# LiyaoTang/contrastBoundary

Hardware: AMD Instinct MI355X
Metric: points/sec through KNN+group+KPConv+CBL block, S3DIS N=40960 K=16 (higher is better)
Workload: dtype f32

## Files before the change

### contrastboundary_amd/csrc/knn_grid.hip

```cpp
#include "cbl_common.h"
#include <cstdlib>
#include "grid_core.h"
#include <knn_wave.h>

int cbl_knn_exact_worklist(int b, int m, int K, const float* xyz, const float* new_xyz, const int* offset,
                           const int* new_offset, int* idx, float* dist2,
                           const int* worklist, const int* worklist_count, int max_work, hipStream_t st,
                           const void* grids, const int* cell_start, const void* sorted);

namespace {

constexpr int GRID_MAX_K = 64;
constexpr int CELLS_PER_POINT = 2;
constexpr int CELLS_PER_CLOUD = 64;

struct Workspace {
    CblGrid* grids;
    int* counters;
    unsigned* bbox;
    int* cell_count;
    int* cell_start;
    int* cell_local;
    int* tile_sum;
    int* pt_cell;
// ... 245 lines not shown
    sort_cx<LEX>(d, i, l8, lane, PermRowMir());    sort_cx<LEX>(d, i, l4, lane, PermSwzXor4());  sort_cx<LEX>(d, i, l2, lane, PermQuadXor2());
    sort_cx<LEX>(d, i, l1, lane, PermQuadXor1());
    sort_cx<LEX>(d, i, l16, lane, PermSwzMir32()); sort_cx<LEX>(d, i, l8, lane, PermRowRor8());  sort_cx<LEX>(d, i, l4, lane, PermSwzXor4());
    sort_cx<LEX>(d, i, l2, lane, PermQuadXor2());  sort_cx<LEX>(d, i, l1, lane, PermQuadXor1());
    sort_cx<LEX>(d, i, l32, lane, PermMir64());    sort_cx<LEX>(d, i, l16, lane, PermSwzXor16()); sort_cx<LEX>(d, i, l8, lane, PermRowRor8());
    sort_cx<LEX>(d, i, l4, lane, PermSwzXor4());   sort_cx<LEX>(d, i, l2, lane, PermQuadXor2()); sort_cx<LEX>(d, i, l1, lane, PermQuadXor1());
}
__device__ __forceinline__ float rl_f(float v, int l) { return __int_as_float(__builtin_amdgcn_readlane(__float_as_int(v), l)); }
template <int G> __device__ __forceinline__ float group_min_nonneg(float f)
{
    int v = __float_as_int(f);
    v = min(v, dppx_i<0xB1>(v)); v = min(v, dppx_i<0x4E>(v)); v = min(v, dppx_i<0x141>(v)); v = min(v, dppx_i<0x140>(v));
    if constexpr (G == 32) v = min(v, __builtin_amdgcn_ds_swizzle(v, 0x401f));
    if constexpr (G == 64) v = min(min(__builtin_amdgcn_readlane(v, 0), __builtin_amdgcn_readlane(v, 16)),
                                   min(__builtin_amdgcn_readlane(v, 32), __builtin_amdgcn_readlane(v, 48)));
    return __int_as_float(v);
}

template <int G, bool SELF, bool LEX>
__global__ __launch_bounds__(256) void knn_grid_group_kernel(int b, int m, int K, const float* __restrict__ new_xyz,
                                                             const int* __restrict__ offset, const int* __restrict__ new_offset,
                                                             const CblGrid* __restrict__ grids, const int* __restrict__ cell_start,
                                                             const float4* __restrict__ sorted, int* __restrict__ idx, float* __restrict__ dist2,
                                                             int* __restrict__ worklist, int* __restrict__ counters, int set_exact)
{
    constexpr int QPW = 64 / G;
    using mask_t = unsigned long long;
    const int lane = threadIdx.x & 63;
    const int gl = lane & (G - 1);
    const int grp = lane / G;
    const int wave_global = (blockIdx.x * 256 + threadIdx.x) >> 6;
    const int t = wave_global * QPW + grp;
    const bool live = t < m;
    const int tt = live ? t : m - 1;

    int q; float qx, qy, qz;
    if (SELF) { const float4 s = sorted[tt]; q = __float_as_int(s.w); qx = s.x; qy = s.y; qz = s.z; }
    else      { q = tt; qx = new_xyz[3 * q]; qy = new_xyz[3 * q + 1]; qz = new_xyz[3 * q + 2]; }
    const int c = cbl_cloud_of(q, SELF ? offset : new_offset, b);
    const CblGrid g = grids[c];
    const float uqx = cbl_u(qx, g.ox, g.inv_cs), uqy = cbl_u(qy, g.oy, g.inv_cs), uqz = cbl_u(qz, g.oz, g.inv_cs);
    const int cx = cbl_cell_coord(uqx, g.nx), cy = cbl_cell_coord(uqy, g.ny), cz = cbl_cell_coord(uqz, g.nz);

    float ed = INFINITY; int ei = -1;
    float rejmin = INFINITY;
    int evict = 0x7f800000;
    const int last_src = ((lane & ~(G - 1)) + K - 1) << 2;
    bool done = !live;

    int rs9 = 0, re9 = 0;
    if (!done && gl < 9) {
        const int o = (int)((0xa82091645ull >> (4 * gl)) & 0xFull);
        const int y = cy + (o & 3) - 1, z = cz + (o >> 2) - 1;
        if (y >= 0 && y < g.ny && z >= 0 && z < g.nz) {
            const int row = g.cell_base + g.nx * (y + g.ny * z);
            rs9 = cell_start[row + max(cx - 1, 0)]; re9 = cell_start[row + min(cx + 1, g.nx - 1) + 1];
        }
    }
    const int grp_src = (lane & ~(G - 1)) << 2;

    for (int r = 1;; r++) {
        const int side = 2 * r + 1;
        for (int ri = 0; ri < side * side; ri++) {
            int dy, dz;
            if (r == 1) { const int o = (int)((0xa82091645ull >> (4 * ri)) & 0xFull); dy = (o & 3) - 1; dz = (o >> 2) - 1; }
            else        { dz = ri / side - r; dy = ri % side - r; }
            {
                const bool full = (r == 1) || dz == -r || dz == r || dy == -r || dy == r;
                const int nseg = full ? 1 : 2;
                for (int sg = 0; sg < nseg; sg++) {
                    int x0, x1;
                    if (full) { x0 = max(cx - r, 0); x1 = min(cx + r, g.nx - 1); }
                    else      { x0 = x1 = sg ? cx + r : cx - r; }
                    const int y = cy + dy, z = cz + dz;
                    int s = 0, e = 0;
                    if (r == 1) {
                        s = __builtin_amdgcn_ds_bpermute(grp_src + (ri << 2), rs9); e = __builtin_amdgcn_ds_bpermute(grp_src + (ri << 2), re9);
                    } else if (!done && y >= 0 && y < g.ny && z >= 0 && z < g.nz && x0 >= 0 && x1 <= g.nx - 1) {
                        const int row = g.cell_base + g.nx * (y + g.ny * z);
                        s = cell_start[row + x0]; e = cell_start[row + x1 + 1];
                    }
                    for (int p = s; __any(p < e); p += G) {
                        const int pi = p + gl;
                        float d2 = INFINITY; int ci = -1;
                        if (pi < e) {
                            const float4 v = sorted[pi];
                            d2 = cbl_dist2(qx, qy, qz, v.x, v.y, v.z);
                            ci = __float_as_int(v.w);
                        }
                        const float worst = __int_as_float(__builtin_amdgcn_ds_bpermute(last_src, __float_as_int(ed)));
                        const unsigned worst_i = LEX ? (unsigned)__builtin_amdgcn_ds_bpermute(last_src, ei) : 0u;
                        const bool pass = d2 < worst || (LEX && d2 == worst && (unsigned)ci < worst_i);
                        rejmin = __int_as_float(min(__float_as_int(rejmin), pass ? 0x7f800000 : __float_as_int(d2)));
                        if constexpr (!LEX && G <= 32) {
                            unsigned gm = (unsigned)(__ballot(pass) >> (grp * G)) & (G == 32 ? ~0u : ((1u << G) - 1u));
                            const int d2i = __float_as_int(d2);
                            auto step = [&]() {
                                const bool has = gm != 0;
                                const int l = kw_ffbl(gm);
                                gm &= gm - 1;
                                const int src = (l << 2) + grp * (G * 4);
                                int dci = __builtin_amdgcn_ds_bpermute(src, d2i); const int ic = __builtin_amdgcn_ds_bpermute(src, ci);
                                dci = has ? dci : 0x7f800000;
                                const int edi = __float_as_int(ed);
                                int pdi = dpp_shr1_zero<G>(edi), pidx = dpp_shr1_zero<G>(ei);
                                if (G == 32) pdi = gl ? pdi : 0;
                                evict = min(evict, max(edi, dci));
                                ei = (edi > dci) ? ((pdi > dci) ? pidx : ic) : ei;
                                ed = __int_as_float(min(edi, max(pdi, dci)));
                            };
                            while (__any(gm != 0)) {
                                step();
                                if (!__any(gm != 0)) break;
                                step();
                            }
                        } else {
                        mask_t gm = (__ballot(pass) >> (grp * G)) & (G == 64 ? ~0ull : ((1ull << G) - 1ull));
                        while (__any(gm != 0)) {
                            const bool has = gm != 0;
                            const int l = has ? __builtin_ctzll(gm) : 0;
                            gm &= gm - 1;
                            float dc = __shfl(d2, l, G); int ic = __shfl(ci, l, G);
                            if (!has) { dc = INFINITY; ic = -1; }
                            const float pd = dpp_shr1_f<G>(ed); const int pidx = dpp_shr1_i<G>(ei);
                            const bool gt = ed > dc || (LEX && ed == dc && (unsigned)ei > (unsigned)ic);
                            const bool left_gt = (gl > 0) && (pd > dc || (LEX && pd == dc && (unsigned)pidx > (unsigned)ic));
                            if (gl == K - 1) rejmin = fminf(rejmin, gt ? ed : dc);
                            if (gt) { if (left_gt) { ed = pd; ei = pidx; } else { ed = dc; ei = ic; } }
                        }
                        }
                    }
                }
            }
        }
        const float bound2 = cbl_outside_bound2(g, uqx, uqy, uqz, cx, cy, cz, r);
        const float worst = __int_as_float(__builtin_amdgcn_ds_bpermute(last_src, __float_as_int(ed)));
        if (!done) done = (bound2 == INFINITY) || (worst < bound2);
        if (__all(done)) break;
    }

    const float worst = __int_as_float(__builtin_amdgcn_ds_bpermute(last_src, __float_as_int(ed)));
    const float rm = group_min_nonneg<G>(fminf(rejmin, gl == K - 1 ? __int_as_float(evict) : INFINITY));
    const float pd = dpp_shr1_f<G>(ed);
    const bool dup = (gl > 0) && (gl < K) && (ed == pd);
    const mask_t dm = (__ballot(dup) >> (grp * G)) & (G == 64 ? ~0ull : ((1ull << G) - 1ull));
    const bool ok = (worst < INFINITY) && (set_exact == 2 || ((rm != worst) && (set_exact ? !(dm & 2ull) : dm == 0)));
    if (live) {
        if (gl < K) { idx[(size_t)q * K + gl] = ei; dist2[(size_t)q * K + gl] = ed; }
        if (!ok && gl == 0) worklist[atomicAdd(counters, 1)] = q;
    }
}


template <bool SELF, bool LEX>
__global__ __launch_bounds__(256) void knn_grid_wave_kernel(int b, int m, int K, const float* __restrict__ new_xyz,
                                                            const int* __restrict__ offset, const int* __restrict__ new_offset,
                                                            const CblGrid* __restrict__ grids, const int* __restrict__ cell_start,
                                                            const float4* __restrict__ sorted, int* __restrict__ idx, float* __restrict__ dist2,
                                                            int* __restrict__ worklist, int* __restrict__ counters, int set_exact,
                                                            int ks, int* __restrict__ idx_n, float* __restrict__ dist2_n,
                                                            int* __restrict__ worklist_n, int set_exact_n, CblCanon canon)
{
    __shared__ float2 slots[4][64];
    if ((int)blockIdx.x < canon.blocks) {
        grid_order_canon_body(canon.n, canon.pt_cell, cell_start, sorted, canon.order, blockIdx.x, canon.blocks);
        return;
    }
    const int lane = threadIdx.x & 63, wv = threadIdx.x >> 6;
    const int t = __builtin_amdgcn_readfirstlane(((int)blockIdx.x - canon.blocks) * 4 + wv);
    if (t >= m) return;
    int q; float qx, qy, qz;
    if (SELF) { const float4 s = sorted[t]; q = __float_as_int(s.w); qx = s.x; qy = s.y; qz = s.z; }
    else      { q = t; qx = new_xyz[3 * q]; qy = new_xyz[3 * q + 1]; qz = new_xyz[3 * q + 2]; }
    q = __builtin_amdgcn_readfirstlane(q);
    const int c = cbl_cloud_of(q, SELF ? offset : new_offset, b);
    const CblGrid g = grids[c];
    const float uqx = cbl_u(qx, g.ox, g.inv_cs), uqy = cbl_u(qy, g.oy, g.inv_cs), uqz = cbl_u(qz, g.oz, g.inv_cs);
    const int cx = cbl_cell_coord(uqx, g.nx), cy = cbl_cell_coord(uqy, g.ny), cz = cbl_cell_coord(uqz, g.nz);

    int rs = 0, rlen = 0;
    if (lane < 9) {
        const int y = cy + lane % 3 - 1, z = cz + lane / 3 - 1;
        if (y >= 0 && y < g.ny && z >= 0 && z < g.nz) {
            const int row = g.cell_base + g.nx * (y + g.ny * z);
            rs = cell_start[row + max(cx - 1, 0)];
            rlen = cell_start[row + min(cx + 1, g.nx - 1) + 1] - rs;
        }
    }
    int pre[9], delta[9], T = 0;
#pragma unroll
    for (int r = 0; r < 9; r++) {
        const int s_r = __builtin_amdgcn_readlane(rs, r), l_r = __builtin_amdgcn_readlane(rlen, r);
        pre[r] = T; delta[r] = s_r - T; T += l_r;
    }

    float ed = INFINITY; int ei = -1;
    float rejmin = INFINITY;
    bool fast = (T >= K) && (T <= 64 * WV_NB);
    if (fast) {
        float d[WV_NB]; int id[WV_NB];
        int delta_v[9];
#pragma unroll
        for (int r = 0; r < 9; r++) delta_v[r] = kw_in_vgpr(delta[r]);
#pragma unroll
        for (int j0 = 0; j0 < WV_NB; j0 += 4) {
            float4 p[4];
#pragma unroll
            for (int u = 0; u < 4; u++) {
                if ((j0 + u) * 64 < T) {
                    const int v = min((j0 + u) * 64 + lane, T - 1);
                    int dl = delta_v[0];
#pragma unroll
                    for (int r = 1; r < 9; r++) dl = (v >= pre[r]) ? delta_v[r] : dl;
                    p[u] = sorted[v + dl];
                }
            }
#pragma unroll
            for (int u = 0; u < 4; u++) {
                const int j = j0 + u;
                d[j] = INFINITY; id[j] = -1;
                if (j * 64 < T) {
                    const bool in = j * 64 + lane < T;
                    const float dd = cbl_dist2(qx, qy, qz, p[u].x, p[u].y, p[u].z);
                    d[j] = in ? dd : INFINITY; id[j] = in ? __float_as_int(p[u].w) : -1;
                }
            }
        }
        float tau = 3.0e38f;
        if (T > 64) {
            int mxi = 0;
#pragma unroll
            for (int j = 0; j < WV_NB; j++) {
                if ((j + 1) * 64 <= T) mxi = max(mxi, __float_as_int(d[j]));
                else if (j * 64 < T)   mxi = max(mxi, d[j] < INFINITY ? __float_as_int(d[j]) : 0);
            }
            mxi = max(mxi, dppx_i<0xB1>(mxi)); mxi = max(mxi, dppx_i<0x4E>(mxi));
            mxi = max(mxi, dppx_i<0x141>(mxi)); mxi = max(mxi, dppx_i<0x140>(mxi));
            float lo = -1.f, hi = __int_as_float(max(max(__builtin_amdgcn_readlane(mxi, 0), __builtin_amdgcn_readlane(mxi, 16)),
                                                     max(__builtin_amdgcn_readlane(mxi, 32), __builtin_amdgcn_readlane(mxi, 48))));
            const float first = (float)(K + 64) * 0.6f * __builtin_amdgcn_rcpf((float)T);
            fast = false;
            for (int it = 0; it < 40; it++) {
                const float mid = it == 0 ? hi * first : lo + (hi - lo) * 0.5f;
                if (!(mid > lo && mid < hi)) break;
                int cnt = 0;
#pragma unroll
                for (int j = 0; j < WV_NB; j++) if (j * 64 < T) cnt += __popcll(__ballot(d[j] <= mid));
                if (cnt < K) lo = mid; else if (cnt > 64) hi = mid; else { tau = mid; fast = true; break; }
            }
        }
        if (fast) {
            int base = 0;
#pragma unroll
            for (int j = 0; j < WV_NB; j++) {
                if (j * 64 < T) {
                    const bool pass = d[j] <= tau;
                    const unsigned long long mk = __ballot(pass);
                    if (pass) {
                        const int slot = base + __builtin_amdgcn_mbcnt_hi((unsigned)(mk >> 32), __builtin_amdgcn_mbcnt_lo((unsigned)mk, 0));
                        slots[wv][slot] = make_float2(d[j], __int_as_float(id[j]));
                    } else rejmin = fminf(rejmin, d[j]);
                    base += __popcll(mk);
                }
            }
            __builtin_amdgcn_fence(__ATOMIC_RELEASE, "wavefront");
            __builtin_amdgcn_wave_barrier();
            __builtin_amdgcn_fence(__ATOMIC_ACQUIRE, "wavefront");
            float sd = INFINITY; int si = -1;
            if (lane < base) { const float2 v = slots[wv][lane]; sd = v.x; si = __float_as_int(v.y); }
            wave_sort64<LEX>(sd, si, lane);
            if (lane < K) { ed = sd; ei = si; } else rejmin = fminf(rejmin, sd);
        }
    }

    bool done = false;
    int r = 1;
    if (fast) {
        const float bound2 = cbl_outside_bound2(g, uqx, uqy, uqz, cx, cy, cz, 1);
        done = (bound2 == INFINITY) || (rl_f(ed, K - 1) < bound2);
        r = 2;
    }
    for (; !done; r++) {
        const int side = 2 * r + 1;
        for (int ri = 0; ri < side * side; ri++) {
            const int dz = ri / side - r, dy = ri % side - r;
            const bool full = (r == 1) || dz == -r || dz == r || dy == -r || dy == r;
            const int nseg = full ? 1 : 2;
            for (int sg = 0; sg < nseg; sg++) {
                int x0, x1;
                if (full) { x0 = max(cx - r, 0); x1 = min(cx + r, g.nx - 1); }
                else      { x0 = x1 = sg ? cx + r : cx - r; }
                const int y = cy + dy, z = cz + dz;
                int s = 0, e = 0;
                if (y >= 0 && y < g.ny && z >= 0 && z < g.nz && x0 >= 0 && x1 <= g.nx - 1) {
                    const int row = g.cell_base + g.nx * (y + g.ny * z);
                    s = cell_start[row + x0]; e = cell_start[row + x1 + 1];
                }
                s = __builtin_amdgcn_readfirstlane(s); e = __builtin_amdgcn_readfirstlane(e);
                for (int p = s; p < e; p += 64) {
                    const int pi = p + lane;
                    float d2 = INFINITY; int ci = -1;
                    if (pi < e) {
                        const float4 v = sorted[pi];
                        d2 = cbl_dist2(qx, qy, qz, v.x, v.y, v.z);
                        ci = __float_as_int(v.w);
                    }
                    const float worst = rl_f(ed, K - 1); const unsigned worst_i = LEX ? (unsigned)__builtin_amdgcn_readlane(ei, K - 1) : 0u;
                    const bool pass = d2 < worst || (LEX && d2 == worst && (unsigned)ci < worst_i);
                    rejmin = fminf(rejmin, pass ? INFINITY : d2);
                    unsigned long long gm = __ballot(pass);
                    while (gm) {
                        const int l = __builtin_ctzll(gm);
                        gm &= gm - 1;
                        const float dc = rl_f(d2, l); const int ic = __builtin_amdgcn_readlane(ci, l);
                        const float pd = dpp_shr1_f<64>(ed); const int pidx = dpp_shr1_i<64>(ei);
                        const bool gt = ed > dc || (LEX && ed == dc && (unsigned)ei > (unsigned)ic);
                        const bool left_gt = (lane > 0) && (pd > dc || (LEX && pd == dc && (unsigned)pidx > (unsigned)ic));
                        if (lane == K - 1) rejmin = fminf(rejmin, gt ? ed : dc);
                        if (gt) { if (left_gt) { ed = pd; ei = pidx; } else { ed = dc; ei = ic; } }
                    }
                }
            }
        }
        const float bound2 = cbl_outside_bound2(g, uqx, uqy, uqz, cx, cy, cz, r);
        done = (bound2 == INFINITY) || (rl_f(ed, K - 1) < bound2);
    }

    const float worst = rl_f(ed, K - 1);
    const float rm = group_min_nonneg<64>(rejmin);
    const float pd = dpp_shr1_f<64>(ed);
    const bool dup = (lane > 0) && (lane < K) && (ed == pd);
    const bool ok = (worst < INFINITY) && (set_exact == 2 || ((rm != worst) && (set_exact ? !(__ballot(dup) & 2ull) : __ballot(dup) == 0)));
    if (lane < K) { idx[(size_t)q * K + lane] = ei; dist2[(size_t)q * K + lane] = ed; }
    if (!ok && lane == 0) worklist[atomicAdd(counters, 1)] = q;
    if (idx_n) {
        if (lane < ks) { idx_n[(size_t)q * ks + lane] = ei; dist2_n[(size_t)q * ks + lane] = ed; }
        const bool bad = (lane > 0 && lane <= ks && ed == pd && (lane == ks || lane == 1 || !set_exact_n)) || (lane == ks - 1 && !(ed < 1e10f));
        if (__ballot(bad) != 0ull && lane == 0) worklist_n[atomicAdd(counters + 1, 1)] = q;
    }
}

template <int G>
void launch_query(bool self, int b, int m, int K, const float* new_xyz, const int* offset, const int* new_offset, const Workspace& w,
                  int* idx, float* dist2, int set_exact, hipStream_t st)
{
    const long long waves = ((long long)m + (64 / G) - 1) / (64 / G);
    const dim3 grid(cbl_div_up(waves, 4)), block(256);
#define CBL_LAUNCH_GROUP(SELF_, LEX_) hipLaunchKernelGGL((knn_grid_group_kernel<G, SELF_, LEX_>), grid, block, 0, st, b, m, K, new_xyz, offset, new_offset, w.grids, \
                                                         w.cell_start, w.sorted, idx, dist2, w.worklist, w.counters, set_exact)
    if (set_exact == 2) { if (self) CBL_LAUNCH_GROUP(true, true); else CBL_LAUNCH_GROUP(false, true); }
    else                { if (self) CBL_LAUNCH_GROUP(true, false); else CBL_LAUNCH_GROUP(false, false); }
#undef CBL_LAUNCH_GROUP
}


template <int G>
__device__ __forceinline__ unsigned long long group_min_u64(unsigned long long v)
{
#pragma unroll
    for (int s = G / 2; s >= 1; s >>= 1) {
        const unsigned lo = __shfl_xor((unsigned)v, s, G), hi = __shfl_xor((unsigned)(v >> 32), s, G);
        const unsigned long long o = ((unsigned long long)hi << 32) | lo;
        v = o < v ? o : v;
    }
    return v;
}

__device__ __forceinline__ unsigned long long radius_key_lds(int t, int total, int c1, int c2, int c3, int c4, int c5, int c6, int c7, int c8, const int* __restrict__ otab,
                                                              float qx, float qy, float qz, float r2, const float4* __restrict__ sorted)
{
    const bool have = t < total;
    const int r = (t >= c1) + (t >= c2) + (t >= c3) + (t >= c4) + (t >= c5) + (t >= c6) + (t >= c7) + (t >= c8);
    const int o = otab[r];
    const float4 v = sorted[have ? t + o : 0];
    const float d2 = cbl_dist2(qx, qy, qz, v.x, v.y, v.z);
    return (have && d2 < r2) ? (((unsigned long long)__float_as_uint(d2) << 32) | (unsigned)__float_as_int(v.w)) : ~0ull;
}

template <int G, int U>
__global__ __launch_bounds__(256) void radius_group_kernel(int b, int nq, int ns_total, int limit, float r2, const float* __restrict__ queries,
                                                           const int* __restrict__ q_offset, const CblGrid* __restrict__ grids,
                                                           const int* __restrict__ cell_start, const float4* __restrict__ sorted,
                                                           int* __restrict__ out, int* __restrict__ counts, int* __restrict__ max_count)
{
    constexpr int QPW = 64 / G, CAP = 2 * G, NBF = G >= 64 ? 2 : 4;
    using mask_t = unsigned long long;
    using key_t = unsigned long long;
    constexpr key_t NONE = ~0ull;
    __shared__ key_t slots[4 * QPW][CAP];
    __shared__ int otabs[4 * QPW][U][12];
    const int lane = threadIdx.x & 63, gl = lane & (G - 1), grp = lane / G;
    key_t* S = slots[(threadIdx.x >> 6) * QPW + grp];
    const int wave_global = (blockIdx.x * 256 + threadIdx.x) >> 6;
    const mask_t below = (1ull << gl) - 1ull, gmask = G == 64 ? ~0ull : ((1ull << G) - 1ull);
    int q[U]; bool live[U]; float qx[U], qy[U], qz[U];
#pragma unroll
    for (int u = 0; u < U; u++) {
        const int t = (wave_global * QPW + grp) * U + u;
        live[u] = t < nq; q[u] = live[u] ? t : nq - 1;
        qx[u] = queries[3 * q[u]]; qy[u] = queries[3 * q[u] + 1]; qz[u] = queries[3 * q[u] + 2];
    }
    int rs[U], re[U];
#pragma unroll
    for (int u = 0; u < U; u++) {
        const int c = cbl_cloud_of(q[u], q_offset, b);
        const CblGrid g = grids[c];
        const int cx = cbl_cell_coord(cbl_u(qx[u], g.ox, g.inv_cs), g.nx), cy = cbl_cell_coord(cbl_u(qy[u], g.oy, g.inv_cs), g.ny),
                  cz = cbl_cell_coord(cbl_u(qz[u], g.oz, g.inv_cs), g.nz);
        const int x0 = max(cx - 1, 0), x1 = min(cx + 1, g.nx - 1);
        rs[u] = 0; re[u] = 0;
        if (gl < 9) {
            const int y = cy + (gl % 3) - 1, z = cz + (gl / 3) - 1;
            if (live[u] && g.end > g.start && y >= 0 && y < g.ny && z >= 0 && z < g.nz) {
                const int row = g.cell_base + g.nx * (y + g.ny * z);
                rs[u] = cell_start[row + x0]; re[u] = cell_start[row + x1 + 1];
            }
        }
    }
    int c1[U], c2[U], c3[U], c4[U], c5[U], c6[U], c7[U], c8[U], total[U];
#pragma unroll
    for (int u = 0; u < U; u++) {
        int* otab = otabs[(threadIdx.x >> 6) * QPW + grp][u];
        int acc = 0;
#define CBL_ROW(r, cnext) { const int sr = __shfl(rs[u], r, G), er = __shfl(re[u], r, G); if (gl == 0) otab[r] = sr - acc; acc += er - sr; cnext = acc; }
        CBL_ROW(0, c1[u]) CBL_ROW(1, c2[u]) CBL_ROW(2, c3[u]) CBL_ROW(3, c4[u]) CBL_ROW(4, c5[u]) CBL_ROW(5, c6[u]) CBL_ROW(6, c7[u]) CBL_ROW(7, c8[u])
        CBL_ROW(8, total[u])
#undef CBL_ROW
    }
#define CBL_KEY(u, t) radius_key_lds((t), total[u], c1[u], c2[u], c3[u], c4[u], c5[u], c6[u], c7[u], c8[u], otabs[(threadIdx.x >> 6) * QPW + grp][u], qx[u], qy[u], qz[u], r2, sorted)
    key_t first[U][NBF];
#pragma unroll
    for (int u = 0; u < U; u++)
#pragma unroll
        for (int k = 0; k < NBF; k++) first[u][k] = CBL_KEY(u, k * G + gl);
#pragma unroll
    for (int u = 0; u < U; u++) {
        int inside = 0;
        auto collect = [&](key_t key) __attribute__((always_inline)) {
            const bool in_ball = key != NONE;
            const mask_t gm = (__ballot(in_ball) >> (grp * G)) & gmask;
            const int slot = inside + __popcll(gm & below);
            if (in_ball && slot < CAP) S[slot] = key;
            inside += __popcll(gm);
        };
#pragma unroll
        for (int k = 0; k < NBF; k++) collect(first[u][k]);
        for (int t0 = NBF * G; __any(t0 < total[u]); t0 += G) collect(CBL_KEY(u, t0 + gl));
        const bool over = inside > CAP;
        if (!over) {
            const int n = inside;
            const key_t ka = gl < n ? S[gl] : NONE, kb = gl + G < n ? S[gl + G] : NONE;
            int ra = 0, rb = 0;
            for (int k = 0; __any(k < n); k += 4) {
                key_t kk[4];
#pragma unroll
                for (int j = 0; j < 4; j++) kk[j] = S[min(k + j, CAP - 1)];
#pragma unroll
                for (int j = 0; j < 4; j++) {
                    const bool on = k + j < n;
                    ra += (on && kk[j] < ka) ? 1 : 0; rb += (on && kk[j] < kb) ? 1 : 0;
                }
            }
            if (live[u]) {
                if (ka != NONE && ra < limit) out[(size_t)q[u] * limit + ra] = (int)(unsigned)ka;
                if (kb != NONE && rb < limit) out[(size_t)q[u] * limit + rb] = (int)(unsigned)kb;
                if (gl >= n && gl < limit) out[(size_t)q[u] * limit + gl] = ns_total;
            }
        }
        if (__any(over)) {
            key_t prev = 0; bool none_yet = true;
            for (int col = 0; col < limit; col++) {
                key_t best = NONE;
                for (int t0 = 0; __any(over && t0 < total[u]); t0 += G) {
                    const key_t key = CBL_KEY(u, t0 + gl);
                    if ((none_yet || key > prev) && key < best) best = key;
                }
                best = group_min_u64<G>(best);
                if (over && live[u] && gl == 0) out[(size_t)q[u] * limit + col] = best == NONE ? ns_total : (int)(unsigned)best;
                prev = best; none_yet = false;
            }
        }
        if (live[u] && gl == 0) {
            if (counts) counts[q[u]] = inside;
            if (inside > __hip_atomic_load(max_count, __ATOMIC_RELAXED, __HIP_MEMORY_SCOPE_AGENT)) atomicMax(max_count, inside);
        }
    }
#undef CBL_KEY
}

}

int cbl_bbox_keys_launch(int b, int n, const float* xyz, const int* offset, unsigned* bbox, hipStream_t st)
{
    hipLaunchKernelGGL(grid_bbox_kernel, dim3(cbl_grid_for(n, 1024, 512)), dim3(256), 0, st, b, n, xyz, offset, bbox);
    return cbl_status();
}

__global__ __launch_bounds__(256) void grid_init_kernel(int b, int total, int* __restrict__ counters, unsigned* __restrict__ bbox, int* __restrict__ cell_count)
{
    const int i0 = blockIdx.x * 256 + threadIdx.x;
    if (i0 < 64) counters[i0] = 0;
    if (i0 < 6 * b) bbox[i0] = ((i0 % 6) < 3) ? 0xffffffffu : 0u;
    for (int i = i0; i < total; i += gridDim.x * 256) cell_count[i] = 0;
}

int cbl_grid_build(int b, int n, float pts_per_cell, const float* xyz, const int* offset, void* ws, hipStream_t st, int* order_out = nullptr, bool canon_later = false)
{
    Workspace w = carve(ws, b, n, 0);
    const int total = w.ncap + 1, ntiles = (total + SCAN_TILE - 1) / SCAN_TILE;
    hipLaunchKernelGGL(grid_init_kernel, dim3(cbl_grid_for(total, 256, 512)), dim3(256), 0, st, b, total, w.counters, w.bbox, w.cell_count);
    hipLaunchKernelGGL(grid_bbox_kernel, dim3(cbl_grid_for(n, 1024, 512)), dim3(256), 0, st, b, n, xyz, offset, w.bbox);
    hipLaunchKernelGGL(grid_count_kernel, dim3(cbl_grid_for(n, 256)), dim3(256), 0, st, b, n, pts_per_cell, xyz, offset, w.bbox, w.grids, w.pt_cell, w.cell_count);
    hipLaunchKernelGGL(grid_scan_tiles_kernel, dim3(ntiles), dim3(256), 0, st, total, w.cell_count, w.cell_local, w.tile_sum);
    hipLaunchKernelGGL(grid_scatter_kernel, dim3(cbl_grid_for(n, 256)), dim3(256), 2 * sizeof(int) * (size_t)ntiles, st, n, total, ntiles, xyz, w.pt_cell,
                       w.tile_sum, w.cell_local, w.cell_start, w.cell_count, w.sorted, order_out);
    if (order_out && !canon_later)
        hipLaunchKernelGGL(grid_order_canon_kernel, dim3(cbl_grid_for(n, 256)), dim3(256), 0, st, n, w.pt_cell, w.cell_start, w.sorted, order_out);
    return cbl_status();
}

__global__ __launch_bounds__(256) void knn_block_candidates_kernel(int b, int n, const int* __restrict__ offset, const CblGrid* __restrict__ grids,
                                                                   const int* __restrict__ cell_start, const float4* __restrict__ sorted, int* __restrict__ count)
{
    const int t = blockIdx.x * 256 + threadIdx.x;
    if (t >= n) return;
    const float4 s = sorted[t];
    const int q = __float_as_int(s.w);
    const CblGrid g = grids[cbl_cloud_of(q, offset, b)];
    const int cx = cbl_cell_coord(cbl_u(s.x, g.ox, g.inv_cs), g.nx), cy = cbl_cell_coord(cbl_u(s.y, g.oy, g.inv_cs), g.ny), cz = cbl_cell_coord(cbl_u(s.z, g.oz, g.inv_cs), g.nz);
    int T = 0;
    for (int r = 0; r < 9; r++) {
        const int y = cy + r % 3 - 1, z = cz + r / 3 - 1;
        if (y >= 0 && y < g.ny && z >= 0 && z < g.nz) {
            const int row = g.cell_base + g.nx * (y + g.ny * z);
            T += cell_start[row + min(cx + 1, g.nx - 1) + 1] - cell_start[row + max(cx - 1, 0)];
        }
    }
    count[q] = T;
}

int cbl_knn_block_candidates_launch(int b, int n, const int* offset, void* ws, int* count, hipStream_t st)
{
    Workspace w = carve(ws, b, n, n);
    hipLaunchKernelGGL(knn_block_candidates_kernel, dim3(cbl_grid_for(n, 256, 1 << 20)), dim3(256), 0, st, b, n, offset, w.grids, w.cell_start, w.sorted, count);
    return cbl_status();
}

size_t cbl_knn_grid_workspace_bytes(int b, int n, int m, int nsample)
{
    if (nsample > GRID_MAX_K || n < 2048 || b <= 0) return 0;
    if ((long long)CELLS_PER_POINT * n + (long long)CELLS_PER_CLOUD * b > 0x3fffffffLL) return 0;
    return carve(nullptr, b, n, m).bytes;
}

void cbl_knn_grid_scratch(void* ws, int b, int n, int m, int** worklist, int** worklist2, int** zero_counter, const void** grids, const int** cell_start,
                          const void** sorted)
{
    Workspace w = carve(ws, b, n, m);
    *worklist = w.worklist; *worklist2 = w.worklist2; *zero_counter = w.counters + 1;
    *grids = w.grids; *cell_start = w.cell_start; *sorted = w.sorted;
}

int cbl_knn_grid_launch(int b, int n, int m, int nsample, const float* xyz, const float* new_xyz, const int* offset,
                        const int* new_offset, int* idx, float* dist2, void* ws, size_t ws_bytes, int set_exact, hipStream_t st, int* order_out,
                        CblKnnNarrow* narrow)
{
    Workspace w = carve(ws, b, n, m);
    if (ws_bytes < w.bytes) return CBL_ERR_WORKSPACE;
    static const float fill = [] { const char* e = getenv("CBL_KNN_CELL_FILL"); const float v = e ? (float)atof(e) : 0.f; return (v > 0.05f && v < 4.f) ? v : 0.33f; }();
    const bool wave_search = nsample > 16;
    int rc = cbl_grid_build(b, n, fill * (float)(nsample < 4 ? 4 : nsample), xyz, offset, ws, st, order_out, wave_search);
    if (rc) return rc;
    const bool self = (new_xyz == xyz) && (m == n);
    if (wave_search) {
        CblCanon canon = {0, n, w.pt_cell, order_out};
        if (order_out) canon.blocks = (int)cbl_grid_for(n, 256);
        const dim3 grid(cbl_div_up(m, 4) + canon.blocks), block(256);
        const int ks = narrow ? narrow->nsample : 0;
        int* idx_n = narrow ? narrow->idx : nullptr; float* dist2_n = narrow ? narrow->dist2 : nullptr;
        const int set_n = narrow ? narrow->set_exact : 0;
        if (narrow) narrow->fused = true;
#define CBL_LAUNCH_WAVE(SELF_, LEX_) hipLaunchKernelGGL((knn_grid_wave_kernel<SELF_, LEX_>), grid, block, 0, st, b, m, nsample, new_xyz, offset, new_offset, w.grids, \
                                                       w.cell_start, w.sorted, idx, dist2, w.worklist, w.counters, set_exact, ks, idx_n, dist2_n, w.worklist2, set_n, canon)
        if (set_exact == 2) { if (self) CBL_LAUNCH_WAVE(true, true); else CBL_LAUNCH_WAVE(false, true); }
        else                { if (self) CBL_LAUNCH_WAVE(true, false); else CBL_LAUNCH_WAVE(false, false); }
#undef CBL_LAUNCH_WAVE
    }
    else launch_query<16>(self, b, m, nsample, new_xyz, offset, new_offset, w, idx, dist2, set_exact, st);
    rc = cbl_status();
    if (rc) return rc;
    if (narrow && narrow->fused && narrow->defer_replay) return CBL_OK;
    return cbl_knn_exact_worklist(b, m, nsample, xyz, new_xyz, self ? offset : offset, self ? offset : new_offset, idx, dist2,
                                  w.worklist, w.counters, m, st, w.grids, w.cell_start, w.sorted);
}

size_t cbl_radius_workspace_bytes_impl(int b, int ns) { return (b > 0 && ns >= 0) ? carve(nullptr, b, ns, 0).bytes : 0; }

int cbl_radius_launch(int b, int nq, int ns, const float* queries, const float* supports, const int* q_offset, const int* s_offset,
                      float radius, int limit, int* out, int* counts, int* max_count, void* ws, size_t ws_bytes, hipStream_t st, bool grid_is_built)
{
    Workspace w = carve(ws, b, ns, 0);
    if (ws_bytes < w.bytes) return CBL_ERR_WORKSPACE;
    int rc = grid_is_built ? CBL_OK : cbl_grid_build(b, ns, -radius, supports, s_offset, ws, st);
    if (rc) return rc;
    hipError_t e = hipMemsetAsync(max_count, 0, sizeof(int), st);
    if (e != hipSuccess) return (int)e;
    const int G = limit <= 16 ? 16 : limit <= 32 ? 32 : 64;
    const long long waves = ((long long)nq + (64 / G) - 1) / (64 / G);
    const dim3 grid(cbl_div_up(waves, 4)), block(256);
    const float r2 = radius * radius;
    const int ru = (long long)nq / ((64 / G) * 2) >= 49152 ? 2 : 1;
    const long long waves_u = ((long long)nq + (64 / G) * ru - 1) / ((64 / G) * ru);
    const dim3 grid_u(cbl_div_up(waves_u, 4));
#define CBL_RAD(G_, U_) hipLaunchKernelGGL((radius_group_kernel<G_, U_>), grid_u, block, 0, st, b, nq, ns, limit, r2, queries, q_offset, w.grids, w.cell_start, w.sorted, out, counts, max_count)
    if (ru == 2) { if (G == 16) CBL_RAD(16, 2); else if (G == 32) CBL_RAD(32, 2); else CBL_RAD(64, 2); }
    else         { if (G == 16) CBL_RAD(16, 1); else if (G == 32) CBL_RAD(32, 1); else CBL_RAD(64, 1); }
#undef CBL_RAD
    return cbl_status();
}
```

Measured before the change: 147.5 million.

## Process runs of cell-sorted queries per wave and reuse staged neighbor candidates in LDS

In the self-query wave KNN kernel, each wavefront now handles a run of four consecutive cell-sorted queries instead of one. When consecutive queries fall in the same grid cell, the 27-cell neighborhood candidates (up to 512) are fetched once into LDS and reused, which avoids repeated global gathers and cell_start lookups. Selection and sorting move into a shared helper. In exchange it adds 32KB of LDS per block, which may reduce occupancy, and it serializes work within a wave while launching four times fewer waves.

```diff
diff --git a/contrastboundary_amd/csrc/knn_grid.hip b/contrastboundary_amd/csrc/knn_grid.hip
--- a/contrastboundary_amd/csrc/knn_grid.hip
+++ b/contrastboundary_amd/csrc/knn_grid.hip
@@ -421,6 +421,62 @@
 }
 
 
+constexpr int WV_RUN = 4;
+constexpr int WV_CAP = 512;
+constexpr int WV_SNB = WV_CAP / 64;
+static_assert(WV_CAP % 64 == 0 && WV_SNB <= WV_NB && WV_RUN >= 1 && WV_RUN <= 64, "a parked block is a whole number of 64-candidate registers; a run is fetched by one load");
+
+template <int NB, bool LEX>
+__device__ __forceinline__ bool wave_select_sort(const float (&d)[NB], const int (&id)[NB], int T, int K, int lane, float2* __restrict__ slots_w,
+                                                 float& ed, int& ei, float& rejmin)
+{
+    float tau = 3.0e38f;
+    if (T > 64) {
+        int mxi = 0;
+#pragma unroll
+        for (int j = 0; j < NB; j++) {
+            if ((j + 1) * 64 <= T) mxi = max(mxi, __float_as_int(d[j]));
+            else if (j * 64 < T)   mxi = max(mxi, d[j] < INFINITY ? __float_as_int(d[j]) : 0);
+        }
+        mxi = max(mxi, dppx_i<0xB1>(mxi)); mxi = max(mxi, dppx_i<0x4E>(mxi));
+        mxi = max(mxi, dppx_i<0x141>(mxi)); mxi = max(mxi, dppx_i<0x140>(mxi));
+        float lo = -1.f, hi = __int_as_float(max(max(__builtin_amdgcn_readlane(mxi, 0), __builtin_amdgcn_readlane(mxi, 16)),
+                                                 max(__builtin_amdgcn_readlane(mxi, 32), __builtin_amdgcn_readlane(mxi, 48))));
+        const float first = (float)(K + 64) * 0.6f * __builtin_amdgcn_rcpf((float)T);
+        bool found = false;
+        for (int it = 0; it < 40; it++) {
+            const float mid = it == 0 ? hi * first : lo + (hi - lo) * 0.5f;
+            if (!(mid > lo && mid < hi)) break;
+            int cnt = 0;
+#pragma unroll
+            for (int j = 0; j < NB; j++) if (j * 64 < T) cnt += __popcll(__ballot(d[j] <= mid));
+            if (cnt < K) lo = mid; else if (cnt > 64) hi = mid; else { tau = mid; found = true; break; }
+        }
+        if (!found) return false;
+    }
+    int base = 0;
+#pragma unroll
+    for (int j = 0; j < NB; j++) {
+        if (j * 64 < T) {
+            const bool pass = d[j] <= tau;
+            const unsigned long long mk = __ballot(pass);
+            if (pass) {
+                const int slot = base + __builtin_amdgcn_mbcnt_hi((unsigned)(mk >> 32), __builtin_amdgcn_mbcnt_lo((unsigned)mk, 0));
+                slots_w[slot] = make_float2(d[j], __int_as_float(id[j]));
+            } else rejmin = fminf(rejmin, d[j]);
+            base += __popcll(mk);
+        }
+    }
+    __builtin_amdgcn_fence(__ATOMIC_RELEASE, "wavefront");
+    __builtin_amdgcn_wave_barrier();
+    __builtin_amdgcn_fence(__ATOMIC_ACQUIRE, "wavefront");
+    float sd = INFINITY; int si = -1;
+    if (lane < base) { const float2 v = slots_w[lane]; sd = v.x; si = __float_as_int(v.y); }
+    wave_sort64<LEX>(sd, si, lane);
+    if (lane < K) { ed = sd; ei = si; } else rejmin = fminf(rejmin, sd);
+    return true;
+}
+
 template <bool SELF, bool LEX>
 __global__ __launch_bounds__(256) void knn_grid_wave_kernel(int b, int m, int K, const float* __restrict__ new_xyz,
                                                             const int* __restrict__ offset, const int* __restrict__ new_offset,
@@ -430,182 +486,210 @@
                                                             int ks, int* __restrict__ idx_n, float* __restrict__ dist2_n,
                                                             int* __restrict__ worklist_n, int set_exact_n, CblCanon canon)
 {
+    constexpr int RUN = SELF ? WV_RUN : 1;
     __shared__ float2 slots[4][64];
+    __shared__ float4 stage[4][SELF ? WV_CAP : 1];
     if ((int)blockIdx.x < canon.blocks) {
         grid_order_canon_body(canon.n, canon.pt_cell, cell_start, sorted, canon.order, blockIdx.x, canon.blocks);
         return;
     }
-    const int lane = threadIdx.x & 63, wv = threadIdx.x >> 6;
-    const int t = __builtin_amdgcn_readfirstlane(((int)blockIdx.x - canon.blocks) * 4 + wv);
-    if (t >= m) return;
-    int q; float qx, qy, qz;
-    if (SELF) { const float4 s = sorted[t]; q = __float_as_int(s.w); qx = s.x; qy = s.y; qz = s.z; }
-    else      { q = t; qx = new_xyz[3 * q]; qy = new_xyz[3 * q + 1]; qz = new_xyz[3 * q + 2]; }
-    q = __builtin_amdgcn_readfirstlane(q);
-    const int c = cbl_cloud_of(q, SELF ? offset : new_offset, b);
-    const CblGrid g = grids[c];
-    const float uqx = cbl_u(qx, g.ox, g.inv_cs), uqy = cbl_u(qy, g.oy, g.inv_cs), uqz = cbl_u(qz, g.oz, g.inv_cs);
-    const int cx = cbl_cell_coord(uqx, g.nx), cy = cbl_cell_coord(uqy, g.ny), cz = cbl_cell_coord(uqz, g.nz);
-
+    const int lane0 = threadIdx.x & 63, wv = threadIdx.x >> 6;
+    const int t0 = __builtin_amdgcn_readfirstlane((((int)blockIdx.x - canon.blocks) * 4 + wv) * RUN);
+    if (t0 >= m) return;
+    const int nq = min(RUN, m - t0);
+    float4 mine = make_float4(0.f, 0.f, 0.f, 0.f);
+    if (SELF) mine = sorted[t0 + min(lane0, nq - 1)];
+
+    CblGrid g = {};
+    int cx = 0, cy = 0, cz = 0, T = 0, cell_end = t0;
     int rs = 0, rlen = 0;
-    if (lane < 9) {
-        const int y = cy + lane % 3 - 1, z = cz + lane / 3 - 1;
-        if (y >= 0 && y < g.ny && z >= 0 && z < g.nz) {
-            const int row = g.cell_base + g.nx * (y + g.ny * z);
-            rs = cell_start[row + max(cx - 1, 0)];
-            rlen = cell_start[row + min(cx + 1, g.nx - 1) + 1] - rs;
-        }
-    }
-    int pre[9], delta[9], T = 0;
-#pragma unroll
-    for (int r = 0; r < 9; r++) {
-        const int s_r = __builtin_amdgcn_readlane(rs, r), l_r = __builtin_amdgcn_readlane(rlen, r);
-        pre[r] = T; delta[r] = s_r - T; T += l_r;
-    }
-
-    float ed = INFINITY; int ei = -1;
-    float rejmin = INFINITY;
-    bool fast = (T >= K) && (T <= 64 * WV_NB);
-    if (fast) {
-        float d[WV_NB]; int id[WV_NB];
-        int delta_v[9];
-#pragma unroll
-        for (int r = 0; r < 9; r++) delta_v[r] = kw_in_vgpr(delta[r]);
-#pragma unroll
-        for (int j0 = 0; j0 < WV_NB; j0 += 4) {
-            float4 p[4];
-#pragma unroll
-            for (int u = 0; u < 4; u++) {
-                if ((j0 + u) * 64 < T) {
-                    const int v = min((j0 + u) * 64 + lane, T - 1);
-                    int dl = delta_v[0];
-#pragma unroll
-                    for (int r = 1; r < 9; r++) dl = (v >= pre[r]) ? delta_v[r] : dl;
-                    p[u] = sorted[v + dl];
+    bool staged = false;
+
+#pragma unroll 1
+    for (int i = 0; i < nq; i++) {
+        const int t = t0 + i;
+        const int lane = lane0 + kw_in_vgpr(0);
+        int q; float qx, qy, qz;
+        if (SELF) { q = __builtin_amdgcn_readlane(__float_as_int(mine.w), i); qx = rl_f(mine.x, i); qy = rl_f(mine.y, i); qz = rl_f(mine.z, i); }
+        else      { q = t; qx = new_xyz[3 * q]; qy = new_xyz[3 * q + 1]; qz = new_xyz[3 * q + 2]; q = __builtin_amdgcn_readfirstlane(q); }
+
+        if (!SELF || t >= cell_end) {
+            const int c = cbl_cloud_of(q, SELF ? offset : new_offset, b);
+            g = grids[c];
+            cx = cbl_cell_coord(cbl_u(qx, g.ox, g.inv_cs), g.nx); cy = cbl_cell_coord(cbl_u(qy, g.oy, g.inv_cs), g.ny);
+            cz = cbl_cell_coord(cbl_u(qz, g.oz, g.inv_cs), g.nz);
+            cx = __builtin_amdgcn_readfirstlane(cx); cy = __builtin_amdgcn_readfirstlane(cy); cz = __builtin_amdgcn_readfirstlane(cz);
+            rs = 0; rlen = 0;
+            if (lane < 9) {
+                const int y = cy + lane % 3 - 1, z = cz + lane / 3 - 1;
+                if (y >= 0 && y < g.ny && z >= 0 && z < g.nz) {
+                    const int row = g.cell_base + g.nx * (y + g.ny * z);
+                    rs = cell_start[row + max(cx - 1, 0)];
+                    rlen = cell_start[row + min(cx + 1, g.nx - 1) + 1] - rs;
                 }
-            }
-#pragma unroll
-            for (int u = 0; u < 4; u++) {
-                const int j = j0 + u;
+            } else if (SELF && lane == 9) {
+                const int cell = g.cell_base + cx + g.nx * (cy + g.ny * cz);
+                rs = cell_start[cell]; rlen = cell_start[cell + 1];
+            }
+            int pre[9], delta[9];
+            T = 0;
+#pragma unroll
+            for (int r = 0; r < 9; r++) {
+                const int s_r = __builtin_amdgcn_readlane(rs, r), l_r = __builtin_amdgcn_readlane(rlen, r);
+                pre[r] = T; delta[r] = s_r - T; T += l_r;
+            }
+            if (SELF) {
+                const int cs = __builtin_amdgcn_readlane(rs, 9), ce = __builtin_amdgcn_readlane(rlen, 9);
+                cell_end = (cs <= t && t < ce) ? ce : t + 1;
+                staged = (T >= K) && (T <= WV_CAP);
+                if (staged) {
+                    int delta_v[9];
+#pragma unroll
+                    for (int r = 0; r < 9; r++) delta_v[r] = kw_in_vgpr(delta[r]);
+                    float4 p[WV_SNB];
+#pragma unroll
+                    for (int j = 0; j < WV_SNB; j++) {
+                        const int v = min(j * 64 + lane, T - 1);
+                        int dl = delta_v[0];
+#pragma unroll
+                        for (int r = 1; r < 9; r++) dl = (v >= pre[r]) ? delta_v[r] : dl;
+                        p[j] = sorted[v + dl];
+                    }
+#pragma unroll
+                    for (int j = 0; j < WV_SNB; j++) stage[wv][j * 64 + lane] = p[j];
+                    __builtin_amdgcn_fence(__ATOMIC_RELEASE, "wavefront");
+                    __builtin_amdgcn_wave_barrier();
+                    __builtin_amdgcn_fence(__ATOMIC_ACQUIRE, "wavefront");
+                }
+            }
+        }
+        const float uqx = cbl_u(qx, g.ox, g.inv_cs), uqy = cbl_u(qy, g.oy, g.inv_cs), uqz = cbl_u(qz, g.oz, g.inv_cs);
+
+        float ed = INFINITY; int ei = -1;
+        float rejmin = INFINITY;
+        bool fast;
+        if (SELF && staged) {
+            float d[WV_SNB]; int id[WV_SNB];
+#pragma unroll
+            for (int j = 0; j < WV_SNB; j++) {
                 d[j] = INFINITY; id[j] = -1;
                 if (j * 64 < T) {
+                    const float4 p = stage[wv][j * 64 + lane];
                     const bool in = j * 64 + lane < T;
-                    const float dd = cbl_dist2(qx, qy, qz, p[u].x, p[u].y, p[u].z);
-                    d[j] = in ? dd : INFINITY; id[j] = in ? __float_as_int(p[u].w) : -1;
+                    const float dd = cbl_dist2(qx, qy, qz, p.x, p.y, p.z);
+                    d[j] = in ? dd : INFINITY; id[j] = in ? __float_as_int(p.w) : -1;
                 }
             }
-        }
-        float tau = 3.0e38f;
-        if (T > 64) {
-            int mxi = 0;
-#pragma unroll
-            for (int j = 0; j < WV_NB; j++) {
-                if ((j + 1) * 64 <= T) mxi = max(mxi, __float_as_int(d[j]));
-                else if (j * 64 < T)   mxi = max(mxi, d[j] < INFINITY ? __float_as_int(d[j]) : 0);
-            }
-            mxi = max(mxi, dppx_i<0xB1>(mxi)); mxi = max(mxi, dppx_i<0x4E>(mxi));
-            mxi = max(mxi, dppx_i<0x141>(mxi)); mxi = max(mxi, dppx_i<0x140>(mxi));
-            float lo = -1.f, hi = __int_as_float(max(max(__builtin_amdgcn_readlane(mxi, 0), __builtin_amdgcn_readlane(mxi, 16)),
-                                                     max(__builtin_amdgcn_readlane(mxi, 32), __builtin_amdgcn_readlane(mxi, 48))));
-            const float first = (float)(K + 64) * 0.6f * __builtin_amdgcn_rcpf((float)T);
-            fast = false;
-            for (int it = 0; it < 40; it++) {
-                const float mid = it == 0 ? hi * first : lo + (hi - lo) * 0.5f;
-                if (!(mid > lo && mid < hi)) break;
-                int cnt = 0;
-#pragma unroll
-                for (int j = 0; j < WV_NB; j++) if (j * 64 < T) cnt += __popcll(__ballot(d[j] <= mid));
-                if (cnt < K) lo = mid; else if (cnt > 64) hi = mid; else { tau = mid; fast = true; break; }
-            }
-        }
-        if (fast) {
-            int base = 0;
-#pragma unroll
-            for (int j = 0; j < WV_NB; j++) {
-                if (j * 64 < T) {
-                    const bool pass = d[j] <= tau;
-                    const unsigned long long mk = __ballot(pass);
-                    if (pass) {
-                        const int slot = base + __builtin_amdgcn_mbcnt_hi((unsigned)(mk >> 32), __builtin_amdgcn_mbcnt_lo((unsigned)mk, 0));
-                        slots[wv][slot] = make_float2(d[j], __int_as_float(id[j]));
-                    } else rejmin = fminf(rejmin, d[j]);
-                    base += __popcll(mk);
-                }
-            }
-            __builtin_amdgcn_fence(__ATOMIC_RELEASE, "wavefront");
-            __builtin_amdgcn_wave_barrier();
-            __builtin_amdgcn_fence(__ATOMIC_ACQUIRE, "wavefront");
-            float sd = INFINITY; int si = -1;
-            if (lane < base) { const float2 v = slots[wv][lane]; sd = v.x; si = __float_as_int(v.y); }
-            wave_sort64<LEX>(sd, si, lane);
-            if (lane < K) { ed = sd; ei = si; } else rejmin = fminf(rejmin, sd);
-        }
-    }
-
-    bool done = false;
-    int r = 1;
-    if (fast) {
-        const float bound2 = cbl_outside_bound2(g, uqx, uqy, uqz, cx, cy, cz, 1);
-        done = (bound2 == INFINITY) || (rl_f(ed, K - 1) < bound2);
-        r = 2;
-    }
-    for (; !done; r++) {
-        const int side = 2 * r + 1;
-        for (int ri = 0; ri < side * side; ri++) {
-            const int dz = ri / side - r, dy = ri % side - r;
-            const bool full = (r == 1) || dz == -r || dz == r || dy == -r || dy == r;
-            const int nseg = full ? 1 : 2;
-            for (int sg = 0; sg < nseg; sg++) {
-                int x0, x1;
-                if (full) { x0 = max(cx - r, 0); x1 = min(cx + r, g.nx - 1); }
-                else      { x0 = x1 = sg ? cx + r : cx - r; }
-                const int y = cy + dy, z = cz + dz;
-                int s = 0, e = 0;
-                if (y >= 0 && y < g.ny && z >= 0 && z < g.nz && x0 >= 0 && x1 <= g.nx - 1) {
-                    const int row = g.cell_base + g.nx * (y + g.ny * z);
-                    s = cell_start[row + x0]; e = cell_start[row + x1 + 1];
-                }
-                s = __builtin_amdgcn_readfirstlane(s); e = __builtin_amdgcn_readfirstlane(e);
-                for (int p = s; p < e; p += 64) {
-                    const int pi = p + lane;
-                    float d2 = INFINITY; int ci = -1;
-                    if (pi < e) {
-                        const float4 v = sorted[pi];
-                        d2 = cbl_dist2(qx, qy, qz, v.x, v.y, v.z);
-                        ci = __float_as_int(v.w);
-                    }
-                    const float worst = rl_f(ed, K - 1); const unsigned worst_i = LEX ? (unsigned)__builtin_amdgcn_readlane(ei, K - 1) : 0u;
-                    const bool pass = d2 < worst || (LEX && d2 == worst && (unsigned)ci < worst_i);
-                    rejmin = fminf(rejmin, pass ? INFINITY : d2);
-                    unsigned long long gm = __ballot(pass);
-                    while (gm) {
-                        const int l = __builtin_ctzll(gm);
-                        gm &= gm - 1;
-                        const float dc = rl_f(d2, l); const int ic = __builtin_amdgcn_readlane(ci, l);
-                        const float pd = dpp_shr1_f<64>(ed); const int pidx = dpp_shr1_i<64>(ei);
-                        const bool gt = ed > dc || (LEX && ed == dc && (unsigned)ei > (unsigned)ic);
-                        const bool left_gt = (lane > 0) && (pd > dc || (LEX && pd == dc && (unsigned)pidx > (unsigned)ic));
-                        if (lane == K - 1) rejmin = fminf(rejmin, gt ? ed : dc);
-                        if (gt) { if (left_gt) { ed = pd; ei = pidx; } else { ed = dc; ei = ic; } }
+            fast = wave_select_sort<WV_SNB, LEX>(d, id, T, K, lane, slots[wv], ed, ei, rejmin);
+        } else {
+            fast = (T >= K) && (T <= 64 * WV_NB);
+            if (fast) {
+                float d[WV_NB]; int id[WV_NB];
+                int pre[9], delta[9];
+                {
+                    int acc = 0;
+#pragma unroll
+                    for (int r = 0; r < 9; r++) {
+                        const int s_r = __builtin_amdgcn_readlane(rs, r), l_r = __builtin_amdgcn_readlane(rlen, r);
+                        pre[r] = acc; delta[r] = s_r - acc; acc += l_r;
                     }
                 }
-            }
-        }
-        const float bound2 = cbl_outside_bound2(g, uqx, uqy, uqz, cx, cy, cz, r);
-        done = (bound2 == INFINITY) || (rl_f(ed, K - 1) < bound2);
-    }
-
-    const float worst = rl_f(ed, K - 1);
-    const float rm = group_min_nonneg<64>(rejmin);
-    const float pd = dpp_shr1_f<64>(ed);
-    const bool dup = (lane > 0) && (lane < K) && (ed == pd);
-    const bool ok = (worst < INFINITY) && (set_exact == 2 || ((rm != worst) && (set_exact ? !(__ballot(dup) & 2ull) : __ballot(dup) == 0)));
-    if (lane < K) { idx[(size_t)q * K + lane] = ei; dist2[(size_t)q * K + lane] = ed; }
-    if (!ok && lane == 0) worklist[atomicAdd(counters, 1)] = q;
-    if (idx_n) {
-        if (lane < ks) { idx_n[(size_t)q * ks + lane] = ei; dist2_n[(size_t)q * ks + lane] = ed; }
-        const bool bad = (lane > 0 && lane <= ks && ed == pd && (lane == ks || lane == 1 || !set_exact_n)) || (lane == ks - 1 && !(ed < 1e10f));
-        if (__ballot(bad) != 0ull && lane == 0) worklist_n[atomicAdd(counters + 1, 1)] = q;
+                int delta_v[9];
+#pragma unroll
+                for (int r = 0; r < 9; r++) delta_v[r] = kw_in_vgpr(delta[r]);
+#pragma unroll
+                for (int j0 = 0; j0 < WV_NB; j0 += 4) {
+                    float4 p[4];
+#pragma unroll
+                    for (int u = 0; u < 4; u++) {
+                        if ((j0 + u) * 64 < T) {
+                            const int v = min((j0 + u) * 64 + lane, T - 1);
+                            int dl = delta_v[0];
+#pragma unroll
+                            for (int r = 1; r < 9; r++) dl = (v >= pre[r]) ? delta_v[r] : dl;
+                            p[u] = sorted[v + dl];
+                        }
+                    }
+#pragma unroll
+                    for (int u = 0; u < 4; u++) {
+                        const int j = j0 + u;
+                        d[j] = INFINITY; id[j] = -1;
+                        if (j * 64 < T) {
+                            const bool in = j * 64 + lane < T;
+                            const float dd = cbl_dist2(qx, qy, qz, p[u].x, p[u].y, p[u].z);
+                            d[j] = in ? dd : INFINITY; id[j] = in ? __float_as_int(p[u].w) : -1;
+                        }
+                    }
+                }
+                fast = wave_select_sort<WV_NB, LEX>(d, id, T, K, lane, slots[wv], ed, ei, rejmin);
+            }
+        }
+
+        bool done = false;
+        int r = 1;
+        if (fast) {
+            const float bound2 = cbl_outside_bound2(g, uqx, uqy, uqz, cx, cy, cz, 1);
+            done = (bound2 == INFINITY) || (rl_f(ed, K - 1) < bound2);
+            r = 2;
+        }
+        for (; !done; r++) {
+            const int side = 2 * r + 1;
+            for (int ri = 0; ri < side * side; ri++) {
+                const int dz = ri / side - r, dy = ri % side - r;
+                const bool full = (r == 1) || dz == -r || dz == r || dy == -r || dy == r;
+                const int nseg = full ? 1 : 2;
+                for (int sg = 0; sg < nseg; sg++) {
+                    int x0, x1;
+                    if (full) { x0 = max(cx - r, 0); x1 = min(cx + r, g.nx - 1); }
+                    else      { x0 = x1 = sg ? cx + r : cx - r; }
+                    const int y = cy + dy, z = cz + dz;
+                    int s = 0, e = 0;
+                    if (y >= 0 && y < g.ny && z >= 0 && z < g.nz && x0 >= 0 && x1 <= g.nx - 1) {
+                        const int row = g.cell_base + g.nx * (y + g.ny * z);
+                        s = cell_start[row + x0]; e = cell_start[row + x1 + 1];
+                    }
+                    s = __builtin_amdgcn_readfirstlane(s); e = __builtin_amdgcn_readfirstlane(e);
+                    for (int p = s; p < e; p += 64) {
+                        const int pi = p + lane;
+                        float d2 = INFINITY; int ci = -1;
+                        if (pi < e) {
+                            const float4 v = sorted[pi];
+                            d2 = cbl_dist2(qx, qy, qz, v.x, v.y, v.z);
+                            ci = __float_as_int(v.w);
+                        }
+                        const float worst = rl_f(ed, K - 1); const unsigned worst_i = LEX ? (unsigned)__builtin_amdgcn_readlane(ei, K - 1) : 0u;
+                        const bool pass = d2 < worst || (LEX && d2 == worst && (unsigned)ci < worst_i);
+                        rejmin = fminf(rejmin, pass ? INFINITY : d2);
+                        unsigned long long gm = __ballot(pass);
+                        while (gm) {
+                            const int l = __builtin_ctzll(gm);
+                            gm &= gm - 1;
+                            const float dc = rl_f(d2, l); const int ic = __builtin_amdgcn_readlane(ci, l);
+                            const float pd = dpp_shr1_f<64>(ed); const int pidx = dpp_shr1_i<64>(ei);
+                            const bool gt = ed > dc || (LEX && ed == dc && (unsigned)ei > (unsigned)ic);
+                            const bool left_gt = (lane > 0) && (pd > dc || (LEX && pd == dc && (unsigned)pidx > (unsigned)ic));
+                            if (lane == K - 1) rejmin = fminf(rejmin, gt ? ed : dc);
+                            if (gt) { if (left_gt) { ed = pd; ei = pidx; } else { ed = dc; ei = ic; } }
+                        }
+                    }
+                }
+            }
+            const float bound2 = cbl_outside_bound2(g, uqx, uqy, uqz, cx, cy, cz, r);
+            done = (bound2 == INFINITY) || (rl_f(ed, K - 1) < bound2);
+        }
+
+        const float worst = rl_f(ed, K - 1);
+        const float rm = group_min_nonneg<64>(rejmin);
+        const float pd = dpp_shr1_f<64>(ed);
+        const bool dup = (lane > 0) && (lane < K) && (ed == pd);
+        const bool ok = (worst < INFINITY) && (set_exact == 2 || ((rm != worst) && (set_exact ? !(__ballot(dup) & 2ull) : __ballot(dup) == 0)));
+        if (lane < K) { idx[(size_t)q * K + lane] = ei; dist2[(size_t)q * K + lane] = ed; }
+        if (!ok && lane == 0) worklist[atomicAdd(counters, 1)] = q;
+        if (idx_n) {
+            if (lane < ks) { idx_n[(size_t)q * ks + lane] = ei; dist2_n[(size_t)q * ks + lane] = ed; }
+            const bool bad = (lane > 0 && lane <= ks && ed == pd && (lane == ks || lane == 1 || !set_exact_n)) || (lane == ks - 1 && !(ed < 1e10f));
+            if (__ballot(bad) != 0ull && lane == 0) worklist_n[atomicAdd(counters + 1, 1)] = q;
+        }
     }
 }
 
@@ -844,7 +928,7 @@
     if (wave_search) {
         CblCanon canon = {0, n, w.pt_cell, order_out};
         if (order_out) canon.blocks = (int)cbl_grid_for(n, 256);
-        const dim3 grid(cbl_div_up(m, 4) + canon.blocks), block(256);
+        const dim3 grid(cbl_div_up(cbl_div_up(m, self ? WV_RUN : 1), 4) + canon.blocks), block(256);
         const int ks = narrow ? narrow->nsample : 0;
         int* idx_n = narrow ? narrow->idx : nullptr; float* dist2_n = narrow ? narrow->dist2 : nullptr;
         const int set_n = narrow ? narrow->set_exact : 0;
```

After: 152.8 million, median of 6. 3.6% higher.
